# LCJebe/PCReg

Hardware: AMD Instinct MI355X
Metric: KNN Gpairs/s end-to-end (search + filters + RANSAC per step; registrations/s = 1000/ms_per_step) (higher is better)
Workload: dtype f32 (search: f16-split matrix-core candidates, exact f32 re-rank) / f64 (RANSAC)

## Files before the change

pcreg_amd/csrc/ransac.hip:

```cpp
#include "common.hpp"
#include <cfloat>
#include <cstddef>
#include <cstdio>
#include <cstdlib>

namespace pcreg {
namespace {

constexpr int kBlock = 256;
constexpr int kWavesPerBlock = 4;
constexpr int HB = 4;

struct RansacArgs {
    const double* p1; const double* p2; int ld;
    const int32_t* offsets;
    const int32_t* n_dev;
    int n_cap; int iters; int m;
    double thDist; double ratio; int refine; unsigned long long seed;
    const int32_t* sample_idx;
    int hpw;
    int hyp0g;
    double* TF;
    int32_t* cnt1; int32_t* cnt2; unsigned char* has;
    int n_hi;
// ... 817 lines not shown
                    unsigned long long bal = __ballot(in);
                    const int r3 = k3 + __popcll(bal & ((1ull << lane) - 1ull));
                    if (in && r3 < 3) {
#pragma unroll
                        for (int c = 0; c < 6; ++c) s_mom[wave][k][r3 * 6 + c] = q[c];
                    }
                    k3 += __popcll(bal);
                }
            PCREG_TILE_SWEEP_END
            if (want && ch != 3) {
                wave_sum27(acc);
#pragma unroll
                for (int e = 0; e < 27; ++e) if (lane == 0) s_mom[wave][k][e] = acc[e];
            }
        }
        __builtin_amdgcn_wave_barrier();
        {
            const bool in_round = mine && lane >= h0 && lane < h0 + HB;
            if (in_round && pass1) {
                double mom[27];
#pragma unroll
                for (int e = 0; e < 27; ++e) mom[e] = s_mom[wave][lane - h0][e];
                if (c1 == 3) {
                    double A1[3][3], A2[3][3];
#pragma unroll
                    for (int j = 0; j < 3; ++j)
#pragma unroll
                        for (int c = 0; c < 3; ++c) { A1[j][c] = mom[j * 6 + c]; A2[j][c] = mom[j * 6 + 3 + c]; }
                    v2 = fit_3pt(A1, A2, T2);
                } else {
                    v2 = fit_moments(c1, mom, o, T2);
                }
            }
        }
        {
            bool any = false;
#pragma unroll
            for (int k = 0; k < HB; ++k) any |= (__builtin_amdgcn_readlane((int)v2, min(h0 + k, 63)) != 0) && (h0 + k < nh);
            if (__syncthreads_or(any)) {
                double T[HB][12]; int cnt[HB];
#pragma unroll
                for (int k = 0; k < HB; ++k) { bcast_T(T2, min(h0 + k, 63), T[k]); pin_translation_vgpr(T[k]); cnt[k] = 0; }
                PCREG_TILE_SWEEP_BEGIN
#pragma unroll
                    for (int k = 0; k < HB; ++k) if (h0 + k < a.hpw) cnt[k] += __popcll(__ballot((sqdist(q, T[k]) < th) & act));
                PCREG_TILE_SWEEP_END
#pragma unroll
                for (int k = 0; k < HB; ++k) if (lane == h0 + k) c2 = cnt[k];
            }
        }
    }
    if (mine) {
        if (!a.refine) {
            a.cnt1[hyp0 + p] = c1; a.cnt2[hyp0 + p] = 0; a.has[hyp0 + p] = pass1;
            if (pass1) {
#pragma unroll
                for (int k = 0; k < 12; ++k) a.TF[(hyp0 + p) * 12 + k] = T1[k];
            }
        } else {
            const bool keep = v2 && c2 >= thInlr;
            a.cnt1[hyp0 + p] = c1; a.cnt2[hyp0 + p] = v2 ? c2 : 0; a.has[hyp0 + p] = keep;
            if (keep) {
#pragma unroll
                for (int k = 0; k < 12; ++k) a.TF[(hyp0 + p) * 12 + k] = T2[k];
            }
        }
    }
}


constexpr int kSW = 4, kSS = 8;
constexpr int kSPts = kSW * kSS * 64;
constexpr int kSMaxPB = 64;
#ifndef PCREG_MOM_SLOTS
#define PCREG_MOM_SLOTS 44
#endif
constexpr int kStagedMinN = 2049;
constexpr int kMomSlots = PCREG_MOM_SLOTS;
constexpr int kRec = 16;
#ifndef PCREG_SCHUNK
#define PCREG_SCHUNK 32
#endif
constexpr int kSChunk = PCREG_SCHUNK;
constexpr int kBBlk = kSS * 64, kBSeeds = 64, kBBuckets = 16, kBChunk = 4;
struct BCtr {
    int32_t lb;
    int32_t hstar;
    int32_t hist[kBBuckets], cursor[kBBuckets];
    int32_t seed_cnt[kBSeeds];
    unsigned long long stats[3];
    int32_t seed_h[kBSeeds];
};
constexpr int kBCtrClearWords = (int)(offsetof(BCtr, seed_h) / 4);

struct StagedArgs {
    RansacArgs a;
    double* T1; unsigned char* v1; unsigned char* pass1; unsigned char* v2;
    unsigned char* cert;
    double* certq;
    double* bounds;
    void* sel_ctr;
    double* bpart;
    int n_rec_blocks;
    double* mom;
    int32_t* part;
    int pb;
    unsigned long long* masks;
    int nslots_cap;
    double* rec;
    double* mpart;
    uint4* dig;
    int32_t* pass_list;
    int32_t* n_pass;
    unsigned char* dense;
    int use_lane;
    float* c32;
    int n32;
    float* T32a; float* T32b;
    int use_f32;
    float* p32;
    int32_t* perm;
    unsigned char* bkt;
    void* bctr;
};

__device__ __forceinline__ int staged_n(const RansacArgs& a) { return min(a.n_dev ? *a.n_dev : a.n_cap, a.n_cap); }

__device__ __forceinline__ void rs_records_body(const StagedArgs& sa, int block) {
    const RansacArgs& a = sa.a;
    const int n = staged_n(a);
    const int i = block * 256 + threadIdx.x;
    double m1 = 0.0, m2 = 0.0, c1m = 0.0, c2m = 0.0;
    if (i >= n && sa.use_lane && i < sa.nslots_cap * 64) {
        double* r = sa.rec + (size_t)i * kRec;
#pragma unroll
        for (int e = 0; e < kRec; ++e) r[e] = 0.0;
    }
    if (i < n) {
        Pts<false> P{a.p1, a.p2, a.ld, nullptr, n};
        double o[6], q[6];
        P.load(0, o); P.load(i, q);
        m1 = q[0] * q[0] + q[1] * q[1] + q[2] * q[2];
        m2 = q[3] * q[3] + q[4] * q[4] + q[5] * q[5];
        if (sa.use_f32 || sa.use_lane) {
            double v[6];
#pragma unroll
            for (int c = 0; c < 6; ++c) { v[c] = q[c] - o[c]; if (sa.use_f32) sa.c32[(size_t)c * sa.n32 + i] = (float)v[c]; }
            c1m = v[0] * v[0] + v[1] * v[1] + v[2] * v[2];
            c2m = v[3] * v[3] + v[4] * v[4] + v[5] * v[5];
        }
        if (sa.use_lane) {
            const double d0 = q[0] - o[0], d1 = q[1] - o[1], d2 = q[2] - o[2];
            const double m0 = q[3] - o[3], m1_ = q[4] - o[4], m2_ = q[5] - o[5];
            double* r = sa.rec + (size_t)i * kRec;
            r[0] = d0; r[1] = d1; r[2] = d2; r[3] = m0; r[4] = m1_; r[5] = m2_;
            r[6] = m0 * d0; r[7] = m0 * d1; r[8] = m0 * d2;
            r[9] = m1_ * d0; r[10] = m1_ * d1; r[11] = m1_ * d2;
            r[12] = m2_ * d0; r[13] = m2_ * d1; r[14] = m2_ * d2; r[15] = 0.0;
        }
    }
#pragma unroll
    for (int o_ = 32; o_ > 0; o_ >>= 1) {
        m1 = fmax(m1, __shfl_xor(m1, o_)); m2 = fmax(m2, __shfl_xor(m2, o_));
        c1m = fmax(c1m, __shfl_xor(c1m, o_)); c2m = fmax(c2m, __shfl_xor(c2m, o_));
    }
    __shared__ double s_mx[4][4];
    if ((threadIdx.x & 63) == 0) { const int w = threadIdx.x >> 6; s_mx[w][0] = m1; s_mx[w][1] = m2; s_mx[w][2] = c1m; s_mx[w][3] = c2m; }
// ... 285 lines not shown
    __syncthreads();
    for (int pb = blockIdx.x; pb * kSPts < n; pb += gridDim.x) {
        float q[kSS][6];
        const int ibase = pb * kSPts + wave * kSS * 64 + lane;
#pragma unroll
        for (int s = 0; s < kSS; ++s) {
            const int i = ibase + s * 64;
            const bool act = i < n;
            const int ii = act ? i : 0;
#pragma unroll
            for (int c = 0; c < 6; ++c) q[s][c] = sa.c32[(size_t)c * sa.n32 + ii];
            if (!act) q[s][0] = __builtin_nanf("");
        }
        rs_i32x16 RA, RB;
#define PCREG_ROW_LOAD(R, H) { const float* rp_ = T32 + (size_t)min((H), h1 - 1) * 16; asm volatile("s_load_dwordx16 %0, %1, 0x0" : "=&s"(R) : "s"(rp_)); }
#define PCREG_ROW_WAIT(R) asm volatile("s_waitcnt lgkmcnt(0)" : "+s"(R))
#define PCREG_SCORE_HYP(H, R)                                                                                      \
        if ((vmask[((H) - h0) >> 6] >> (((H) - h0) & 63)) & 1ull) {                                \
            float T[12];                                                                                           \
            _Pragma("unroll") for (int k = 0; k < 12; ++k) { const int w_ = R[k]; T[k] = __int_as_float(w_); }                 \
            const int wlo_ = R[12], whi_ = R[13]; const float thlo = __int_as_float(wlo_), thhi = __int_as_float(whi_);          \
            unsigned long long b[kSS], band = 0ull;                                                                \
            _Pragma("unroll") for (int s = 0; s < kSS; ++s) {                                                      \
                const float d = sqdist32(q[s], T);                                                                 \
                b[s] = __ballot(d < thlo);                                                                         \
                band |= __ballot(d <= thhi) ^ b[s];       \
            }                                                                                                      \
            if (band != 0ull) {       \
                double T64[12];       \
                _Pragma("unroll") for (int k = 0; k < 12; ++k) T64[k] = TT[(size_t)(H) * 12 + k];    \
                _Pragma("unroll 1") for (int s = 0; s < kSS; ++s) {       \
                    const int i = ibase + s * 64;                         \
                    const bool act = i < n;                                                                        \
                    const int ii = act ? i : 0;                                                                    \
                    float qq[6];                                                                                   \
                    _Pragma("unroll") for (int c = 0; c < 6; ++c) qq[c] = sa.c32[(size_t)c * sa.n32 + ii];         \
                    if (!act) qq[0] = __builtin_nanf("");                                                          \
                    const float d = sqdist32(qq, T);                                                               \
                    if ((__ballot(d <= thhi) ^ __ballot(d < thlo)) != 0ull) {                     \
                        double p[6];                                                                               \
                        _Pragma("unroll") for (int c = 0; c < 3; ++c) { p[c] = a.p1[ii + (size_t)c * a.ld]; p[3 + c] = a.p2[ii + (size_t)c * a.ld]; } \
                        const unsigned long long bb = __ballot((sqdist(p, T64) < th) & act);                       \
                        _Pragma("unroll") for (int s2 = 0; s2 < kSS; ++s2) if (s2 == s) b[s2] = bb;                \
                    }                                                                                              \
                }                                                                                                  \
            }                                                                                                      \
            int cnt = 0;                                                                                           \
            int mine_lo = 0, mine_hi = 0;                                                                          \
            _Pragma("unroll") for (int s = 0; s < kSS; ++s) {                                                      \
                cnt += __popcll(b[s]);                                                                             \
                if (EMIT) {                                                               \
                    asm volatile("v_writelane_b32 %0, %1, %2" : "+v"(mine_lo) : "s"((int)(unsigned)b[s]), "n"(s)); \
                    asm volatile("v_writelane_b32 %0, %1, %2" : "+v"(mine_hi) : "s"((int)(unsigned)(b[s] >> 32)), "n"(s)); \
                }                                                                                                  \
            }                                                                                                      \
            if (lane == 0) s_cnt[wave][(H) - h0] += cnt;                                                           \
            if (EMIT && lane < kSS)                            \
                sa.masks[(size_t)(H) * sa.nslots_cap + (size_t)pb * (kSPts / 64) + wave * kSS + lane] =            \
                    ((unsigned long long)(unsigned)mine_hi << 32) | (unsigned)mine_lo;                             \
        }
        PCREG_ROW_LOAD(RA, h0)
        PCREG_ROW_WAIT(RA);
        for (int h = h0; h < h1; h += 2) {
            PCREG_ROW_LOAD(RB, h + 1)
            PCREG_SCORE_HYP(h, RA)
            PCREG_ROW_WAIT(RB); PCREG_ROW_LOAD(RA, h + 2)
            if (h + 1 < h1) { PCREG_SCORE_HYP(h + 1, RB) }
            PCREG_ROW_WAIT(RA);
        }
#undef PCREG_SCORE_HYP
#undef PCREG_ROW_WAIT
#undef PCREG_ROW_LOAD
    }
    __syncthreads();
    for (int hl = threadIdx.x; hl < h1 - h0; hl += kSW * 64) {
        int c = 0;
#pragma unroll
        for (int w = 0; w < kSW; ++w) c += s_cnt[w][hl];
        if (acc) { if (c) atomicAdd(&acc[h0 + hl], c); } else sa.part[(size_t)blockIdx.x * a.iters + h0 + hl] = c;
    }
}


__device__ __forceinline__ void rs_load_block(const StagedArgs& sa, const float* __restrict__ x32, int base, int n, float (&q)[kSS][6]) {
    const int lane = threadIdx.x & 63;
#pragma unroll
    for (int s = 0; s < kSS; ++s) {
        const int i = base + s * 64 + lane;
        const bool act = i < n;
        const int ii = act ? i : 0;
#pragma unroll
        for (int c = 0; c < 6; ++c) q[s][c] = x32[(size_t)c * sa.n32 + ii];
        if (!act) q[s][0] = __builtin_nanf("");
    }
}
__device__ __forceinline__ int rs_block_count(const StagedArgs& sa, const float* __restrict__ x32, const int32_t* __restrict__ perm,
                                              int base, int n, const float (&q)[kSS][6], const float (&T)[12], float thlo, float thhi,
                                              int h) {
    const RansacArgs& a = sa.a;
    const int lane = threadIdx.x & 63;
    unsigned long long b[kSS], band = 0ull;
#pragma unroll
    for (int s = 0; s < kSS; ++s) {
        const float d = sqdist32(q[s], T);
        b[s] = __ballot(d < thlo);
        band |= __ballot(d <= thhi) ^ b[s];
    }
    if (band != 0ull) {
        double T64[12];
#pragma unroll
        for (int k = 0; k < 12; ++k) T64[k] = a.TF[(size_t)h * 12 + k];
#pragma unroll 1
        for (int s = 0; s < kSS; ++s) {
            const int i = base + s * 64 + lane;
            const bool act = i < n;
            const int ii = act ? i : 0;
            float qq[6];
#pragma unroll
            for (int c = 0; c < 6; ++c) qq[c] = x32[(size_t)c * sa.n32 + ii];
            if (!act) qq[0] = __builtin_nanf("");
            const float d = sqdist32(qq, T);
            if ((__ballot(d <= thhi) ^ __ballot(d < thlo)) != 0ull) {
                const int oi = perm ? perm[ii] : ii;
                double p[6];
#pragma unroll
                for (int c = 0; c < 3; ++c) { p[c] = a.p1[oi + (size_t)c * a.ld]; p[3 + c] = a.p2[oi + (size_t)c * a.ld]; }
                const unsigned long long bb = __ballot((sqdist(p, T64) < a.thDist) & act);
#pragma unroll
                for (int s2 = 0; s2 < kSS; ++s2) if (s2 == s) b[s2] = bb;
            }
        }
    }
    int cnt = 0;
#pragma unroll
    for (int s = 0; s < kSS; ++s) cnt += __popcll(b[s]);
    return cnt;
}

__device__ __forceinline__ unsigned long long rs_cnt1_key(const StagedArgs& sa, int lo, int hi) {
    unsigned long long key = 0ull;
#pragma unroll 4
    for (int p = lo + (int)(threadIdx.x & 63); p < hi; p += 64) {
        const unsigned char v = sa.v2[p];
        const unsigned long long k = ((unsigned long long)(unsigned)sa.a.cnt1[p] << 32) | (unsigned)(0xFFFFFFFFu - (unsigned)p);
        key = v && k > key ? k : key;
    }
#pragma unroll
    for (int o = 32; o > 0; o >>= 1) { const unsigned long long ot = __shfl_xor(key, o); key = ot > key ? ot : key; }
    return key;
}
__device__ __forceinline__ int rs_key_index(unsigned long long key) { return key ? (int)(0xFFFFFFFFu - (unsigned)(key & 0xFFFFFFFFull)) : -1; }

__device__ __forceinline__ int rs_order_bucket(float d, float th) {
    if (!(d < th) || !(th < 3.0e38f)) return 0;
    const int k = (int)((th - d) * ((float)(kBBuckets - 1) / th));
    return 1 + min(kBBuckets - 2, max(k, 0));
}

__global__ __launch_bounds__(256) void rs_bprep_kernel(StagedArgs sa, int n_seed_wg, int S, int nbc) {
    const RansacArgs& a = sa.a;
    BCtr* bc = (BCtr*)sa.bctr;
    const int n = staged_n(a);
    const int lane = threadIdx.x & 63, wave = threadIdx.x >> 6;
    if ((int)blockIdx.x < n_seed_wg) {
        const int u = blockIdx.x * 4 + wave;
        const int s = u / nbc, blk = u - s * nbc;
        if (s >= S || (blk > 0 && blk * kBBlk >= n)) return;
        const int lo = (int)((long long)s * a.iters / S), hi = (int)((long long)(s + 1) * a.iters / S);
        const int h = rs_key_index(rs_cnt1_key(sa, lo, hi));
        if (blk == 0 && lane == 0) bc->seed_h[s] = h;
        if (h < 0 || blk * kBBlk >= n) return;
        float q[kSS][6];
        rs_load_block(sa, sa.c32, blk * kBBlk, n, q);
        const float* row = sa.T32b + (size_t)h * 16;
        float T[12];
#pragma unroll
        for (int k = 0; k < 12; ++k) T[k] = row[k];
        const int c = rs_block_count(sa, sa.c32, nullptr, blk * kBBlk, n, q, T, row[12], row[13], h);
        if (lane == 0 && c) atomicAdd(&bc->seed_cnt[s], c);
        return;
    }
    const int ob = blockIdx.x - n_seed_wg;
    __shared__ unsigned long long s_key[4];
    __shared__ int s_hist[kBBuckets];
    if (threadIdx.x < kBBuckets) s_hist[threadIdx.x] = 0;
    {
        unsigned long long k = 0ull;
        const int n4 = a.iters >> 2;
        const int4* c4 = (const int4*)a.cnt1;
        const unsigned* v4 = (const unsigned*)sa.v2;
#pragma unroll 4
        for (int p4 = threadIdx.x; p4 < n4; p4 += 256) {
            const int4 c = c4[p4];
            const unsigned v = v4[p4];
            const int cc[4] = {c.x, c.y, c.z, c.w};
#pragma unroll
            for (int e = 0; e < 4; ++e) {
                const unsigned p = (unsigned)(4 * p4 + e);
                const unsigned long long ke = ((v >> (8 * e)) & 0xFFu) ? ((unsigned long long)(unsigned)cc[e] << 32) | (0xFFFFFFFFu - p) : 0ull;
                k = ke > k ? ke : k;
            }
        }
        for (int p = 4 * n4 + (int)threadIdx.x; p < a.iters; p += 256)
            if (sa.v2[p]) { const unsigned long long ke = ((unsigned long long)(unsigned)a.cnt1[p] << 32) | (0xFFFFFFFFu - (unsigned)p); k = ke > k ? ke : k; }
#pragma unroll
        for (int o = 32; o > 0; o >>= 1) { const unsigned long long ot = __shfl_xor(k, o); k = ot > k ? ot : k; }
        if (lane == 0) s_key[wave] = k;
    }
    __syncthreads();
    unsigned long long key = s_key[0];
#pragma unroll
    for (int w = 1; w < 4; ++w) key = s_key[w] > key ? s_key[w] : key;
    const int hs = rs_key_index(key);
    if (ob == 0) {
        if (threadIdx.x == 0) bc->hstar = hs;
        if ((int)threadIdx.x >= S && threadIdx.x < kBSeeds) bc->seed_h[threadIdx.x] = -1;
    }
    const int i = ob * 256 + threadIdx.x;
    if (i < n) {
        int bk = 0;
        if (hs >= 0) {
            float q[6], T[12];
#pragma unroll
            for (int c = 0; c < 6; ++c) q[c] = sa.c32[(size_t)c * sa.n32 + i];
#pragma unroll
            for (int k = 0; k < 12; ++k) T[k] = sa.T32b[(size_t)hs * 16 + k];
            bk = rs_order_bucket(sqdist32(q, T), (float)a.thDist);
        }
        sa.bkt[i] = (unsigned char)bk;
        atomicAdd(&s_hist[bk], 1);
    }
    __syncthreads();
    if (threadIdx.x < kBBuckets && s_hist[threadIdx.x]) atomicAdd(&bc->hist[threadIdx.x], s_hist[threadIdx.x]);
}

__global__ __launch_bounds__(256) void rs_bscatter_kernel(StagedArgs sa) {
    BCtr* bc = (BCtr*)sa.bctr;
    const int n = staged_n(sa.a);
    __shared__ int s_cnt[kBBuckets], s_off[kBBuckets];
    if (threadIdx.x < kBBuckets) s_cnt[threadIdx.x] = 0;
    __syncthreads();
    const int i = blockIdx.x * 256 + threadIdx.x;
    int bk = 0, r = 0;
    if (i < n) { bk = sa.bkt[i]; r = atomicAdd(&s_cnt[bk], 1); }
    __syncthreads();
    if (threadIdx.x < kBBuckets) {
        int off = 0;
        for (int k = 0; k < (int)threadIdx.x; ++k) off += bc->hist[k];
        s_off[threadIdx.x] = off + (s_cnt[threadIdx.x] ? atomicAdd(&bc->cursor[threadIdx.x], s_cnt[threadIdx.x]) : 0);
    }
    __syncthreads();
    if (i < n) {
        const int pos = s_off[bk] + r;
#pragma unroll
        for (int c = 0; c < 6; ++c) sa.p32[(size_t)c * sa.n32 + pos] = sa.c32[(size_t)c * sa.n32 + i];
        sa.perm[pos] = i;
    }
}

template <int C>
__global__ __launch_bounds__(64) void rs_bounded_kernel(StagedArgs sa, unsigned long long* __restrict__ stats) {
    static_assert(C >= 1 && C <= 64, "one lane per refit");
    const RansacArgs& a = sa.a;
    BCtr* bc = (BCtr*)sa.bctr;
    const int n = staged_n(a);
    const int lane = threadIdx.x;
    const int thInlr = matlab_round_i(a.ratio * (double)n);
    const int h0 = blockIdx.x * C, hl = h0 + lane;
    const bool mine = lane < C && hl < a.iters;
    const int nb = (n + kBBlk - 1) / kBBlk;
    const int sh = bc->seed_h[lane], sc = bc->seed_cnt[lane];
    int lb = sh >= 0 ? sc : 0;
#pragma unroll
    for (int o = 32; o > 0; o >>= 1) lb = max(lb, __shfl_xor(lb, o));
    bool live = mine && sa.v2[hl] != 0;
    const unsigned long long exist = __ballot(live);
    int seedc = -1;
    for (int s = 0; s < kBSeeds; ++s) {
        const int hs = __builtin_amdgcn_readlane(sh, s), cs = __builtin_amdgcn_readlane(sc, s);
        if (hs == hl) seedc = cs;
    }
    if (live && seedc >= 0) { a.cnt2[hl] = seedc; live = false; }
    unsigned long long active = __ballot(live);
    const unsigned long long seeded = exist & ~active;
    float comp[14];
#pragma unroll
    for (int k = 0; k < 14; ++k) comp[k] = live ? sa.T32b[(size_t)hl * 16 + k] : 0.0f;
    int in_v = 0;
    unsigned long long units = 0ull;
    float qa[kSS][6], qb[kSS][6];
    if (active != 0ull && nb > 0) rs_load_block(sa, sa.p32, 0, n, qa);
    int lbr0 = lb, lbr1 = lb;
    auto step = [&](int blk, const float (&cur)[kSS][6], float (&nxt)[kSS][6], int& lbr) {
        if (blk + 1 < nb) rs_load_block(sa, sa.p32, (blk + 1) * kBBlk, n, nxt);
        const int base = blk * kBBlk;
        for (unsigned long long m = active; m != 0ull; m &= m - 1ull) {
            const int j = __builtin_ctzll(m);
            float T[12];
#pragma unroll
            for (int k = 0; k < 12; ++k) T[k] = __int_as_float(__builtin_amdgcn_readlane(__float_as_int(comp[k]), j));
            const float thlo = __int_as_float(__builtin_amdgcn_readlane(__float_as_int(comp[12]), j));
            const float thhi = __int_as_float(__builtin_amdgcn_readlane(__float_as_int(comp[13]), j));
            const int c = rs_block_count(sa, sa.p32, sa.perm, base, n, cur, T, thlo, thhi, h0 + j);
            in_v += lane == j ? c : 0;
        }
        units += (unsigned long long)__popcll(active);
        lb = max(lb, lbr);
        lbr = __hip_atomic_load(&bc->lb, __ATOMIC_RELAXED, __HIP_MEMORY_SCOPE_AGENT);
        const int out_v = min(n, base + kBBlk) - in_v;
        const bool stop = ((active >> lane) & 1ull) && out_v > n - lb && (in_v >= thInlr || out_v > n - thInlr);
        if (stop) a.cnt2[hl] = in_v >= thInlr ? thInlr : 0;
        active &= ~__ballot(stop);
    };
    for (int blk = 0; blk < nb && active != 0ull; blk += 2) {
        step(blk, qa, qb, lbr0);
        if (blk + 1 < nb && active != 0ull) step(blk + 1, qb, qa, lbr1);
    }
    const bool full = (active >> lane) & 1ull;
    if (full) a.cnt2[hl] = in_v;
    int mx = full ? in_v : 0;
#pragma unroll
    for (int o = 32; o > 0; o >>= 1) mx = max(mx, __shfl_xor(mx, o));
    if (lane == 0 && active != 0ull && mx > lb) __hip_atomic_fetch_max(&bc->lb, mx, __ATOMIC_RELAXED, __HIP_MEMORY_SCOPE_AGENT);
    if (stats && lane == 0) {
        if (blockIdx.x == 0) atomicAdd(&stats[0], 1ull);
        atomicAdd(&stats[1], units + (unsigned long long)__popcll(seeded) * (unsigned long long)nb);
        atomicAdd(&stats[2], (unsigned long long)__popcll(exist) * (unsigned long long)nb);
    }
}

constexpr int kHB32 = 4;
typedef unsigned rs_u32x2 __attribute__((ext_vector_type(2)));

template <int CTRL>
__device__ __forceinline__ double dpp_f64(double v) {
    const int lo = __builtin_amdgcn_mov_dpp(__double2loint(v), CTRL, 0xF, 0xF, false);
    const int hi = __builtin_amdgcn_mov_dpp(__double2hiint(v), CTRL, 0xF, 0xF, false);
    return __hiloint2double(hi, lo);
}
__device__ __forceinline__ double swap32_add(double A, double B) {
    const rs_u32x2 r0 = __builtin_amdgcn_permlane32_swap((unsigned)__double2loint(A), (unsigned)__double2loint(B), false, false);
    const rs_u32x2 r1 = __builtin_amdgcn_permlane32_swap((unsigned)__double2hiint(A), (unsigned)__double2hiint(B), false, false);
    return __hiloint2double((int)r1[0], (int)r0[0]) + __hiloint2double((int)r1[1], (int)r0[1]);
}
__device__ __forceinline__ double swap16_add(double A, double B) {
    const rs_u32x2 r0 = __builtin_amdgcn_permlane16_swap((unsigned)__double2loint(A), (unsigned)__double2loint(B), false, false);
    const rs_u32x2 r1 = __builtin_amdgcn_permlane16_swap((unsigned)__double2hiint(A), (unsigned)__double2hiint(B), false, false);
    return __hiloint2double((int)r1[0], (int)r0[0]) + __hiloint2double((int)r1[1], (int)r0[1]);
}
__device__ __forceinline__ double wave_sum15_scatter(const double (&v)[15]) {
    const int lane = threadIdx.x & 63;
    double r1[8], r2[4], r3[2];
#pragma unroll
    for (int j = 0; j < 8; ++j) r1[j] = swap32_add(v[j], j < 7 ? v[j < 7 ? 8 + j : 14] : 0.0);
#pragma unroll
    for (int j = 0; j < 4; ++j) r2[j] = swap16_add(r1[j], r1[4 + j]);
    const bool b3 = lane & 8, b2 = lane & 4;
#pragma unroll
    for (int j = 0; j < 2; ++j) r3[j] = (b3 ? r2[2 + j] : r2[j]) + dpp_f64<0x128>(b3 ? r2[j] : r2[2 + j]);
    double r = (b2 ? r3[1] : r3[0]) + dpp_f64<0x1B>(dpp_f64<0x141>(b2 ? r3[0] : r3[1]));
    r += dpp_f64<0x4E>(r);
    r += dpp_f64<0xB1>(r);
    return r;
}
__device__ __forceinline__ void mom15_add(double (&m)[15], const double (&q)[6]) {
    m[0] += q[0]; m[1] += q[1]; m[2] += q[2]; m[3] += q[3]; m[4] += q[4]; m[5] += q[5];
    m[6]  = fma(q[3], q[0], m[6]);  m[7]  = fma(q[3], q[1], m[7]);  m[8]  = fma(q[3], q[2], m[8]);
    m[9]  = fma(q[4], q[0], m[9]);  m[10] = fma(q[4], q[1], m[10]); m[11] = fma(q[4], q[2], m[11]);
    m[12] = fma(q[5], q[0], m[12]); m[13] = fma(q[5], q[1], m[13]); m[14] = fma(q[5], q[2], m[14]);
}
__device__ bool fit_moments15(int N, const double (&mom)[15], const double (&o)[6], double (&T)[12]) {
    if (N < 4) return false;
    const double inv = 1.0 / (double)N;
    const double cdp[3] = {mom[0] * inv, mom[1] * inv, mom[2] * inv};
    const double cmp_[3] = {mom[3] * inv, mom[4] * inv, mom[5] * inv};
    double H[3][3];
#pragma unroll
    for (int i = 0; i < 3; ++i)
#pragma unroll
        for (int j = 0; j < 3; ++j) H[i][j] = mom[6 + i * 3 + j] - (double)N * cmp_[i] * cdp[j];
    const double cd[3] = {cdp[0] + o[0], cdp[1] + o[1], cdp[2] + o[2]};
    const double cm[3] = {cmp_[0] + o[3], cmp_[1] + o[4], cmp_[2] + o[5]};
    return polar_to_T(H, cd, cm, T);
}
__device__ __forceinline__ double ld_coherent(const double* p) { return __hip_atomic_load(p, __ATOMIC_RELAXED, __HIP_MEMORY_SCOPE_AGENT); }

struct Hyp32Lds { const double* c64; const float* c32; int np; int ns; };
typedef float rs_f32x2 __attribute__((ext_vector_type(2)));

__device__ __forceinline__ float sqdist32r(const float (&q)[6], const float (&T)[12]) {
    float ux = q[0] - T[9], uy = q[1] - T[10], uz = q[2] - T[11];
    ux = __builtin_fmaf(q[5], -T[2], ux); uy = __builtin_fmaf(q[5], -T[5], uy); uz = __builtin_fmaf(q[5], -T[8], uz);
    ux = __builtin_fmaf(q[4], -T[1], ux); uy = __builtin_fmaf(q[4], -T[4], uy); uz = __builtin_fmaf(q[4], -T[7], uz);
    ux = __builtin_fmaf(q[3], -T[0], ux); uy = __builtin_fmaf(q[3], -T[3], uy); uz = __builtin_fmaf(q[3], -T[6], uz);
    return __builtin_fmaf(uz, uz, __builtin_fmaf(uy, uy, ux * ux));
}
__device__ __forceinline__ rs_f32x2 sqdist32r_x2(const rs_f32x2 (&q)[6], const rs_f32x2 (&P)[6]) {
    rs_f32x2 ux, uy, uz, d;
    asm("v_pk_add_f32 %0, %4, %10 op_sel_hi:[1,0] neg_lo:[0,1] neg_hi:[0,1]\n\t"
        "v_pk_add_f32 %1, %5, %10 op_sel:[0,1] op_sel_hi:[1,1] neg_lo:[0,1] neg_hi:[0,1]\n\t"
        "v_pk_add_f32 %2, %6, %11 op_sel_hi:[1,0] neg_lo:[0,1] neg_hi:[0,1]\n\t"
        "v_pk_fma_f32 %0, %9, %11, %0 op_sel:[0,1,0] op_sel_hi:[1,1,1] neg_lo:[0,1,0] neg_hi:[0,1,0]\n\t"
        "v_pk_fma_f32 %1, %9, %12, %1 op_sel_hi:[1,0,1] neg_lo:[0,1,0] neg_hi:[0,1,0]\n\t"
        "v_pk_fma_f32 %2, %9, %12, %2 op_sel:[0,1,0] op_sel_hi:[1,1,1] neg_lo:[0,1,0] neg_hi:[0,1,0]\n\t"
        "v_pk_fma_f32 %0, %8, %13, %0 op_sel_hi:[1,0,1] neg_lo:[0,1,0] neg_hi:[0,1,0]\n\t"
        "v_pk_fma_f32 %1, %8, %13, %1 op_sel:[0,1,0] op_sel_hi:[1,1,1] neg_lo:[0,1,0] neg_hi:[0,1,0]\n\t"
        "v_pk_fma_f32 %2, %8, %14, %2 op_sel_hi:[1,0,1] neg_lo:[0,1,0] neg_hi:[0,1,0]\n\t"
        "v_pk_fma_f32 %0, %7, %14, %0 op_sel:[0,1,0] op_sel_hi:[1,1,1] neg_lo:[0,1,0] neg_hi:[0,1,0]\n\t"
        "v_pk_fma_f32 %1, %7, %15, %1 op_sel_hi:[1,0,1] neg_lo:[0,1,0] neg_hi:[0,1,0]\n\t"
        "v_pk_fma_f32 %2, %7, %15, %2 op_sel:[0,1,0] op_sel_hi:[1,1,1] neg_lo:[0,1,0] neg_hi:[0,1,0]\n\t"
        "v_pk_mul_f32 %3, %0, %0\n\t"
// ... 1204 lines not shown
    if (ws_bytes < need) { set_error("ransac workspace too small: %zu < %zu", ws_bytes, need); return PCREG_E_WORKSPACE; }
    size_t h = (size_t)o.iterNum * (size_t)B;
    RansacArgs a{};
    a.p1 = p1; a.p2 = p2; a.ld = ld; a.offsets = offsets; a.n_dev = n_dev; a.n_cap = n_cap;
    a.iters = o.iterNum; a.m = o.minPtNum; a.thDist = o.thDist; a.ratio = o.thInlrRatio;
    a.refine = o.REFINE != 0; a.seed = o.seed; a.sample_idx = sample_idx_dev; a.hyp0g = hyp_begin;
    a.n_hi = 0x7FFFFFFF; a.n_lo = -1;
    a.TF = lay.TF; a.cnt1 = lay.cnt1; a.cnt2 = lay.cnt2; a.has = lay.has;
    long long total = (long long)o.iterNum * B;
    void* sel_ctr = nullptr;
    SelFinish sel_fin{nullptr, nullptr, 0};
    bool fold_finish = false;
    if (debug_flag(kDbgRansacResidentF64) && n_cap > 0 && (size_t)n_cap * 48 <= (offsets ? (size_t)152 * 1024 : (size_t)64 * 1024)) {
        size_t lds = (size_t)n_cap * 48;
        int hpw = 64;
        while (hpw > 8 && total / hpw < 256LL * 4 * 2) hpw >>= 1;
        a.hpw = hpw;
        if (offsets && lds > 64 * 1024) { lds = 32 * 1024; a.n_hi = (int)(lds / 48); }
        const int pb4 = hpw * kWavesPerBlock;
        hipLaunchKernelGGL(ransac_hyp_kernel, dim3((o.iterNum + pb4 - 1) / pb4, B), dim3(kBlock), lds, st, a);
    } else if (n_cap > 0 && n_cap <= (offsets ? kHyp32BatchCap : kHyp32Classes[kHyp32NClasses - 1])) {
        int hpw = 64;
        while (hpw > 8 && total / hpw < 256LL * 4 * 2) hpw >>= 1;
        a.hpw = hpw;
        a.msc = lay.msc;
        const int c = n_cap <= kHyp32Classes[0] ? 0 : 1;
        a.n_lo = -1; a.n_hi = std::min(n_cap, kHyp32Classes[c]);
        const int nw = kHyp32Waves[c], per_block = hpw * nw;
        const dim3 grid((o.iterNum + per_block - 1) / per_block, B);
        const int rc = nw == 8 ? launch_hyp32<8>(a, grid, hyp32_lds_bytes(a.n_hi, nw), st) : launch_hyp32<16>(a, grid, hyp32_lds_bytes(a.n_hi, nw), st);
        if (rc != PCREG_OK) return rc;
        const int lo = a.n_hi;
        if (n_cap > lo) {
            a.n_lo = lo; a.n_hi = -1;
            const int pb4 = hpw * kWavesPerBlock;
            hipLaunchKernelGGL(ransac_hyp_kernel, dim3((o.iterNum + pb4 - 1) / pb4, B), dim3(kBlock), 0, st, a);
        }
    } else if (B == 1 && !offsets && staged_pays(n_cap, o.iterNum) && !debug_flag(kDbgRansacFused)) {
        StagedArgs sa = lay.sa;
        sel_ctr = sa.sel_ctr;
        sa.use_lane = a.refine && !debug_flag(kDbgRansacNoLane);
        sa.use_f32 = !debug_flag(kDbgRansacF64Score);
        int pb = (n_cap + kSPts - 1) / kSPts; if (pb > kSMaxPB) pb = kSMaxPB; if (pb < 1) pb = 1;
        sa.pb = pb;
        int hpw = (int)((total + 250LL * kTW - 1) / (250LL * kTW));
        if (hpw < 1) hpw = 1;
        if (hpw > 16) hpw = 16;
        a.hpw = hpw;
        sa.a = a;
        const int it = o.iterNum;
        const dim3 sgrid(pb, (it + kSChunk - 1) / kSChunk);
        const int n_fit = (it + 255) / 256;
        hipLaunchKernelGGL(rs_stage1_kernel, dim3((unsigned)(n_fit + sa.n_rec_blocks)), dim3(256), 0, st, sa, n_fit);
        const int n_t32 = (it + 255) / 256, n_dig = sa.use_lane ? (int)staged_slots_cap(n_cap) * 2 : 0;
        hipLaunchKernelGGL(rs_stage2_kernel, dim3((unsigned)(n_t32 + n_dig)), dim3(256), 0, st, sa, (const double*)sa.T1, sa.T32a, n_t32, sa.dig);
        if (sa.use_f32) {
            if (sa.use_lane)
                hipLaunchKernelGGL(rs_score32_kernel<true>, sgrid, dim3(kSW * 64), 0, st, sa, (const double*)sa.T1, (const float*)sa.T32a, (const unsigned char*)sa.v1, (int32_t*)nullptr);
            else
                hipLaunchKernelGGL(rs_score32_kernel<false>, sgrid, dim3(kSW * 64), 0, st, sa, (const double*)sa.T1, (const float*)sa.T32a, (const unsigned char*)sa.v1, (int32_t*)nullptr);
        } else if (sa.use_lane) {
            hipLaunchKernelGGL(rs_score_kernel<true>, sgrid, dim3(kSW * 64), 0, st, sa, (const double*)sa.T1, (const unsigned char*)sa.v1);
        } else {
            hipLaunchKernelGGL(rs_score_kernel<false>, sgrid, dim3(kSW * 64), 0, st, sa, (const double*)sa.T1, (const unsigned char*)sa.v1);
        }
        hipLaunchKernelGGL(rs_pass1_kernel, dim3((it + 255) / 256), dim3(256), 0, st, sa);
        if (a.refine) {
            if (sa.use_lane)
                hipLaunchKernelGGL(rs_moments_mfma_kernel, dim3((it + kMmWaves * kMmRows - 1) / (kMmWaves * kMmRows), (unsigned)staged_chunks_cap(n_cap)), dim3(kMmWaves * 64), 0, st, sa,
                                   (const uint4*)sa.dig, (const unsigned long long*)sa.masks);
            hipLaunchKernelGGL(rs_moments_kernel, dim3((it + hpw * kTW - 1) / (hpw * kTW)), dim3(kTBlock), 0, st, sa);
            hipLaunchKernelGGL(rs_fit2_kernel, dim3((it + 63) / 64), dim3(64), 0, st, sa);
            fold_finish = !part && n_cap <= kSelBlocks * kSelPerThread * kSelThreads;
            const int p2mode = debug_flag(kDbgRansacPass2);
            const bool bounded = fold_finish && sa.use_f32 && !iter_inl_ref && p2mode != 1 && (p2mode == 2 || bounded_pays(n_cap, it));
            if (bounded) {
                const int S = std::min(kBSeeds, it), nbc = (n_cap + kBBlk - 1) / kBBlk;
                const int n_seed_wg = (S * nbc + 3) / 4, n_ord_wg = (n_cap + 255) / 256;
                unsigned long long* stats = ransac_stats_dev();
                hipLaunchKernelGGL(rs_bprep_kernel, dim3((unsigned)(n_seed_wg + n_ord_wg)), dim3(256), 0, st, sa, n_seed_wg, S, nbc);
                hipLaunchKernelGGL(rs_bscatter_kernel, dim3((unsigned)n_ord_wg), dim3(256), 0, st, sa);
#ifdef PCREG_EXPERIMENTS
                const int dbg = PCREG_EXP_ENV("PCREG_RANSAC_DEBUG", 0), chunk = PCREG_EXP_ENV("PCREG_RANSAC_BCHUNK", kBChunk);
                unsigned long long* kst = dbg ? ((BCtr*)sa.bctr)->stats : stats;
                if (chunk == 8) hipLaunchKernelGGL(rs_bounded_kernel<8>, dim3((unsigned)((it + 7) / 8)), dim3(64), 0, st, sa, kst);
                else if (chunk == 2) hipLaunchKernelGGL(rs_bounded_kernel<2>, dim3((unsigned)((it + 1) / 2)), dim3(64), 0, st, sa, kst);
                else hipLaunchKernelGGL(rs_bounded_kernel<kBChunk>, dim3((unsigned)((it + kBChunk - 1) / kBChunk)), dim3(64), 0, st, sa, kst);
                if (dbg) {
                    unsigned long long u[3] = {0, 0, 0};
                    PCREG_HIP(hipMemcpyAsync(u, kst, sizeof u, hipMemcpyDeviceToHost, st));
                    PCREG_HIP(hipStreamSynchronize(st));
                    fprintf(stderr, "[pcreg] ransac bounded pass 2: iters=%d n_cap=%d chunk=%d (refit, block) units scanned %llu of %llu (%.4f)\n", it, n_cap,
                            chunk == 8 || chunk == 2 ? chunk : kBChunk, u[1], u[2], u[2] ? (double)u[1] / (double)u[2] : 0.0);
                }
#else
                hipLaunchKernelGGL(rs_bounded_kernel<kBChunk>, dim3((unsigned)((it + kBChunk - 1) / kBChunk)), dim3(64), 0, st, sa, stats);
#endif
            } else if (sa.use_f32)
                hipLaunchKernelGGL(rs_score32_kernel<false>, sgrid, dim3(kSW * 64), 0, st, sa, (const double*)a.TF, (const float*)sa.T32b, (const unsigned char*)sa.v2,
                                   fold_finish ? a.cnt2 : (int32_t*)nullptr);
            else
                hipLaunchKernelGGL(rs_score_kernel<false>, sgrid, dim3(kSW * 64), 0, st, sa, (const double*)a.TF, (const unsigned char*)sa.v2);
            if (fold_finish) { sel_fin.part = sa.use_f32 ? nullptr : sa.part; sel_fin.v2 = sa.v2; sel_fin.pb = sa.pb; }
            else hipLaunchKernelGGL(rs_finish_kernel, dim3((it + 255) / 256), dim3(256), 0, st, sa);
        }
    } else {
        int hpw = (int)((total + 250LL * kTW - 1) / (250LL * kTW));
        if (hpw < 1) hpw = 1;
        if (hpw > 16) hpw = 16;
        a.hpw = hpw;
        int per_block = hpw * kTW;
        dim3 grid((o.iterNum + per_block - 1) / per_block, B);
        hipLaunchKernelGGL(ransac_hyp_tiled_kernel, grid, dim3(kTBlock), 0, st, a);
    }
    PCREG_HIP(hipGetLastError());
    if (sel_ctr && !part && n_cap <= kSelBlocks * kSelPerThread * kSelThreads) {
        int per_block = 4 * kSelThreads;
        if ((n_cap + per_block - 1) / per_block > kSelBlocks) per_block = ((n_cap + kSelBlocks - 1) / kSelBlocks + kSelThreads - 1) / kSelThreads * kSelThreads;
        const int nb = std::max(1, (n_cap + per_block - 1) / per_block);
        hipLaunchKernelGGL(ransac_select_multi_kernel, dim3(nb), dim3(kSelThreads), 0, st, a, out, inlier_idx, (SelCtr*)sel_ctr, per_block, sel_fin);
    }
    else if (n_cap >= 8192) hipLaunchKernelGGL(ransac_select_kernel<1024>, dim3(B), dim3(1024), 0, st, a, out, inlier_idx, part);
    else hipLaunchKernelGGL(ransac_select_kernel<kBlock>, dim3(B), dim3(kBlock), 0, st, a, out, inlier_idx, part);
    PCREG_HIP(hipGetLastError());
    if (iter_inl) PCREG_HIP(hipMemcpyAsync(iter_inl, a.cnt1, h * sizeof(int32_t), hipMemcpyDeviceToDevice, st));
    if (iter_inl_ref) PCREG_HIP(hipMemcpyAsync(iter_inl_ref, a.cnt2, h * sizeof(int32_t), hipMemcpyDeviceToDevice, st));
    return PCREG_OK;
}

int launch_ransac(const double* p1, const double* p2, int ld, const int32_t* offsets, const int32_t* n_dev,
                  int n_cap, int B, const pcreg_ransac_opts& o, const int32_t* sample_idx_dev,
                  pcreg_dev_ransac_result* out, int32_t* inlier_idx, int32_t* iter_inl, int32_t* iter_inl_ref,
                  void* ws, size_t ws_bytes, hipStream_t st) {
    return launch_ransac_impl(p1, p2, ld, offsets, n_dev, n_cap, B, o, sample_idx_dev, out, inlier_idx, iter_inl, iter_inl_ref,
                              ws, ws_bytes, st, 0, nullptr);
}

int launch_ransac_partial(const double* p1, const double* p2, int ld, const int32_t* n_dev, int n_cap,
                          const pcreg_ransac_opts& o, const int32_t* sample_idx_dev, int hyp_begin, int hyp_count,
                          pcreg_dev_ransac_part* part, void* ws, size_t ws_bytes, hipStream_t st) {
    PCREG_ARG(hyp_begin >= 0 && hyp_count >= 0 && hyp_begin + hyp_count <= o.iterNum);
    if (hyp_count == 0) { PCREG_HIP(hipMemsetAsync(part, 0, sizeof(pcreg_dev_ransac_part), st)); return PCREG_OK; }
    pcreg_ransac_opts ol = o;
    ol.iterNum = hyp_count;
    return launch_ransac_impl(p1, p2, ld, nullptr, n_dev, n_cap, 1, ol, sample_idx_dev, nullptr, nullptr, nullptr, nullptr,
                              ws, ws_bytes, st, hyp_begin, part);
}

int launch_ransac_finish(const double* p1, const double* p2, int ld, const int32_t* n_dev, int n_cap,
                         const pcreg_ransac_opts& o, const pcreg_dev_ransac_part* combined,
                         pcreg_dev_ransac_result* out, int32_t* inlier_idx, hipStream_t st, int n_parts) {
    PCREG_ARG(n_parts >= 1);
    RansacArgs a{};
    a.p1 = p1; a.p2 = p2; a.ld = ld; a.n_dev = n_dev; a.n_cap = n_cap; a.thDist = o.thDist; a.ratio = o.thInlrRatio;
    if (n_cap >= 8192) hipLaunchKernelGGL(ransac_finish_kernel<1024>, dim3(1), dim3(1024), 0, st, a, combined, n_parts, out, inlier_idx);
    else hipLaunchKernelGGL(ransac_finish_kernel<kBlock>, dim3(1), dim3(kBlock), 0, st, a, combined, n_parts, out, inlier_idx);
    PCREG_HIP(hipGetLastError());
    return PCREG_OK;
}

int launch_estimate_transform(const double* p1, const double* p2, int n, int ld, double* T16_dev,
                              int32_t* empty_dev, hipStream_t st) {
    hipLaunchKernelGGL(estimate_transform_kernel, dim3(1), dim3(64), 0, st, p1, p2, n, ld, T16_dev, empty_dev);
    PCREG_HIP(hipGetLastError());
    return PCREG_OK;
}

int launch_refine_by_distance(const double* p1, const double* p2, const int32_t* n_dev, int cap, int ld, double maxDist,
                              double* T16_dev, int32_t* info_dev, hipStream_t st) {
    hipLaunchKernelGGL(refine_by_distance_kernel, dim3(1), dim3(64), 0, st, p1, p2, n_dev, cap, ld, maxDist, T16_dev, info_dev);
    PCREG_HIP(hipGetLastError());
    return PCREG_OK;
}

int launch_estimate_transform_indexed(const double* p1, const double* p2, int ld, const int32_t* idx, int32_t idx_base, const int32_t* n_idx_dev,
                                      int cap, double* T16_dev, int32_t* info_dev, hipStream_t st) {
    hipLaunchKernelGGL(estimate_transform_indexed_kernel, dim3(1), dim3(64), 0, st, p1, p2, ld, idx, (int)idx_base, n_idx_dev, cap, T16_dev, info_dev);
    PCREG_HIP(hipGetLastError());
    return PCREG_OK;
// ... 23 lines not shown
```

Measured before the change: 123,700.

## Split bounded RANSAC scoring blocks across four waves per workgroup

The bounded pass-2 kernel now runs four waves per workgroup. Each wave scores a different 512-point block for the same small set of refit hypotheses, and per-round counts and the lower bound are combined through shared memory with a barrier. Point loads are also vectorised to float4 per lane, which reorders rows within a block. This targets latency in what was a single-wave serial scan, at the cost of a barrier each round and coarser early-stop granularity, since all four blocks are scanned before a stop check.

```diff
diff --git a/pcreg_amd/csrc/ransac.hip b/pcreg_amd/csrc/ransac.hip
--- a/pcreg_amd/csrc/ransac.hip
+++ b/pcreg_amd/csrc/ransac.hip
@@ -923,7 +923,8 @@
 #define PCREG_SCHUNK 32
 #endif
 constexpr int kSChunk = PCREG_SCHUNK;
-constexpr int kBBlk = kSS * 64, kBSeeds = 64, kBBuckets = 16, kBChunk = 4;
+constexpr int kBBlk = kSS * 64, kBSeeds = 64, kBBuckets = 16, kBChunk = 4, kBWaves = 4;
+constexpr bool kBPrefetch = true;
 struct BCtr {
     int32_t lb;
     int32_t hstar;
@@ -1375,16 +1376,20 @@
 }
 
 
+__device__ __forceinline__ int rs_block_row(int s, int lane) { return 256 * (s >> 2) + 4 * lane + (s & 3); }
 __device__ __forceinline__ void rs_load_block(const StagedArgs& sa, const float* __restrict__ x32, int base, int n, float (&q)[kSS][6]) {
+    static_assert(kSS == 8 && kSPts % kBBlk == 0, "two float4 per lane and coordinate");
     const int lane = threadIdx.x & 63;
 #pragma unroll
-    for (int s = 0; s < kSS; ++s) {
-        const int i = base + s * 64 + lane;
-        const bool act = i < n;
-        const int ii = act ? i : 0;
-#pragma unroll
-        for (int c = 0; c < 6; ++c) q[s][c] = x32[(size_t)c * sa.n32 + ii];
-        if (!act) q[s][0] = __builtin_nanf("");
+    for (int g = 0; g < 2; ++g) {
+        const int i0 = base + 256 * g + 4 * lane;
+#pragma unroll
+        for (int c = 0; c < 6; ++c) {
+            const float4 v = ((const float4*)(x32 + (size_t)c * sa.n32 + base + 256 * g))[lane];
+            q[4 * g][c] = v.x; q[4 * g + 1][c] = v.y; q[4 * g + 2][c] = v.z; q[4 * g + 3][c] = v.w;
+        }
+#pragma unroll
+        for (int e = 0; e < 4; ++e) if (i0 + e >= n) q[4 * g + e][0] = __builtin_nanf("");
     }
 }
 __device__ __forceinline__ int rs_block_count(const StagedArgs& sa, const float* __restrict__ x32, const int32_t* __restrict__ perm,
@@ -1405,7 +1410,7 @@
         for (int k = 0; k < 12; ++k) T64[k] = a.TF[(size_t)h * 12 + k];
 #pragma unroll 1
         for (int s = 0; s < kSS; ++s) {
-            const int i = base + s * 64 + lane;
+            const int i = base + rs_block_row(s, lane);
             const bool act = i < n;
             const int ii = act ? i : 0;
             float qq[6];
@@ -1551,17 +1556,21 @@
     }
 }
 
-template <int C>
-__global__ __launch_bounds__(64) void rs_bounded_kernel(StagedArgs sa, unsigned long long* __restrict__ stats) {
+template <int C, int W, bool PF>
+__global__ __launch_bounds__(64 * W) void rs_bounded_kernel(StagedArgs sa, unsigned long long* __restrict__ stats) {
     static_assert(C >= 1 && C <= 64, "one lane per refit");
+    static_assert(W >= 1 && W <= 16, "waves of one workgroup");
     const RansacArgs& a = sa.a;
     BCtr* bc = (BCtr*)sa.bctr;
     const int n = staged_n(a);
-    const int lane = threadIdx.x;
+    const int lane = threadIdx.x & 63, wave = threadIdx.x >> 6;
     const int thInlr = matlab_round_i(a.ratio * (double)n);
     const int h0 = blockIdx.x * C, hl = h0 + lane;
     const bool mine = lane < C && hl < a.iters;
     const int nb = (n + kBBlk - 1) / kBBlk;
+    __shared__ int s_cnt[2][W][C];
+    __shared__ int s_lb[2];
+    __shared__ unsigned long long s_units[W];
     const int sh = bc->seed_h[lane], sc = bc->seed_cnt[lane];
     int lb = sh >= 0 ? sc : 0;
 #pragma unroll
@@ -1573,7 +1582,7 @@
         const int hs = __builtin_amdgcn_readlane(sh, s), cs = __builtin_amdgcn_readlane(sc, s);
         if (hs == hl) seedc = cs;
     }
-    if (live && seedc >= 0) { a.cnt2[hl] = seedc; live = false; }
+    if (live && seedc >= 0) { if (wave == 0) a.cnt2[hl] = seedc; live = false; }
     unsigned long long active = __ballot(live);
     const unsigned long long seeded = exist & ~active;
     float comp[14];
@@ -1582,44 +1591,68 @@
     int in_v = 0;
     unsigned long long units = 0ull;
     float qa[kSS][6], qb[kSS][6];
-    if (active != 0ull && nb > 0) rs_load_block(sa, sa.p32, 0, n, qa);
+    if (PF && active != 0ull && wave < nb) rs_load_block(sa, sa.p32, wave * kBBlk, n, qa);
     int lbr0 = lb, lbr1 = lb;
-    auto step = [&](int blk, const float (&cur)[kSS][6], float (&nxt)[kSS][6], int& lbr) {
-        if (blk + 1 < nb) rs_load_block(sa, sa.p32, (blk + 1) * kBBlk, n, nxt);
-        const int base = blk * kBBlk;
-        for (unsigned long long m = active; m != 0ull; m &= m - 1ull) {
-            const int j = __builtin_ctzll(m);
-            float T[12];
-#pragma unroll
-            for (int k = 0; k < 12; ++k) T[k] = __int_as_float(__builtin_amdgcn_readlane(__float_as_int(comp[k]), j));
-            const float thlo = __int_as_float(__builtin_amdgcn_readlane(__float_as_int(comp[12]), j));
-            const float thhi = __int_as_float(__builtin_amdgcn_readlane(__float_as_int(comp[13]), j));
-            const int c = rs_block_count(sa, sa.p32, sa.perm, base, n, cur, T, thlo, thhi, h0 + j);
-            in_v += lane == j ? c : 0;
-        }
-        units += (unsigned long long)__popcll(active);
-        lb = max(lb, lbr);
-        lbr = __hip_atomic_load(&bc->lb, __ATOMIC_RELAXED, __HIP_MEMORY_SCOPE_AGENT);
-        const int out_v = min(n, base + kBBlk) - in_v;
+    auto step = [&](int r, float (&cur)[kSS][6], float (&nxt)[kSS][6], int& lbr) {
+        const int blk = W * r + wave, base = blk * kBBlk;
+        if (PF) { if (blk + W < nb) rs_load_block(sa, sa.p32, (blk + W) * kBBlk, n, nxt); }
+        else if (blk < nb) rs_load_block(sa, sa.p32, base, n, cur);
+        int c_v = 0;
+        if (blk < nb) {
+            for (unsigned long long m = active; m != 0ull; m &= m - 1ull) {
+                const int j = __builtin_ctzll(m);
+                float T[12];
+#pragma unroll
+                for (int k = 0; k < 12; ++k) T[k] = __int_as_float(__builtin_amdgcn_readlane(__float_as_int(comp[k]), j));
+                const float thlo = __int_as_float(__builtin_amdgcn_readlane(__float_as_int(comp[12]), j));
+                const float thhi = __int_as_float(__builtin_amdgcn_readlane(__float_as_int(comp[13]), j));
+                const int c = rs_block_count(sa, sa.p32, sa.perm, base, n, cur, T, thlo, thhi, h0 + j);
+                c_v += lane == j ? c : 0;
+            }
+            units += (unsigned long long)__popcll(active);
+        }
+        if (lane < C) s_cnt[r & 1][wave][lane] = c_v;
+        if (wave == 0) {
+            if (lane == 0) s_lb[r & 1] = lbr;
+            lbr = __hip_atomic_load(&bc->lb, __ATOMIC_RELAXED, __HIP_MEMORY_SCOPE_AGENT);
+        }
+        __syncthreads();
+        if (lane < C) {
+#pragma unroll
+            for (int w = 0; w < W; ++w) in_v += s_cnt[r & 1][w][lane];
+        }
+        lb = max(lb, s_lb[r & 1]);
+        const int out_v = min(n, (W * r + W) * kBBlk) - in_v;
         const bool stop = ((active >> lane) & 1ull) && out_v > n - lb && (in_v >= thInlr || out_v > n - thInlr);
-        if (stop) a.cnt2[hl] = in_v >= thInlr ? thInlr : 0;
+        if (stop && wave == 0) a.cnt2[hl] = in_v >= thInlr ? thInlr : 0;
         active &= ~__ballot(stop);
     };
-    for (int blk = 0; blk < nb && active != 0ull; blk += 2) {
-        step(blk, qa, qb, lbr0);
-        if (blk + 1 < nb && active != 0ull) step(blk + 1, qb, qa, lbr1);
+    const int nr = (nb + W - 1) / W;
+    for (int r = 0; r < nr && active != 0ull; r += 2) {
+        step(r, qa, PF ? qb : qa, lbr0);
+        if (r + 1 < nr && active != 0ull) step(r + 1, PF ? qb : qa, qa, lbr1);
     }
     const bool full = (active >> lane) & 1ull;
+    if (lane == 0) s_units[wave] = units;
+    __syncthreads();
+    if (wave != 0) return;
     if (full) a.cnt2[hl] = in_v;
     int mx = full ? in_v : 0;
 #pragma unroll
     for (int o = 32; o > 0; o >>= 1) mx = max(mx, __shfl_xor(mx, o));
     if (lane == 0 && active != 0ull && mx > lb) __hip_atomic_fetch_max(&bc->lb, mx, __ATOMIC_RELAXED, __HIP_MEMORY_SCOPE_AGENT);
     if (stats && lane == 0) {
+        units = 0ull;
+#pragma unroll
+        for (int w = 0; w < W; ++w) units += s_units[w];
         if (blockIdx.x == 0) atomicAdd(&stats[0], 1ull);
         atomicAdd(&stats[1], units + (unsigned long long)__popcll(seeded) * (unsigned long long)nb);
         atomicAdd(&stats[2], (unsigned long long)__popcll(exist) * (unsigned long long)nb);
     }
+}
+template <int C, int W, bool PF>
+static void rs_bounded_launch(const StagedArgs& sa, int it, unsigned long long* stats, hipStream_t st) {
+    hipLaunchKernelGGL((rs_bounded_kernel<C, W, PF>), dim3((unsigned)((it + C - 1) / C)), dim3(64 * W), 0, st, sa, stats);
 }
 
 constexpr int kHB32 = 4;
@@ -2990,19 +3023,24 @@
                 hipLaunchKernelGGL(rs_bscatter_kernel, dim3((unsigned)n_ord_wg), dim3(256), 0, st, sa);
 #ifdef PCREG_EXPERIMENTS
                 const int dbg = PCREG_EXP_ENV("PCREG_RANSAC_DEBUG", 0), chunk = PCREG_EXP_ENV("PCREG_RANSAC_BCHUNK", kBChunk);
+                const int waves = PCREG_EXP_ENV("PCREG_RANSAC_BWAVES", kBWaves), pf = PCREG_EXP_ENV("PCREG_RANSAC_BPREFETCH", kBPrefetch ? 1 : 0);
                 unsigned long long* kst = dbg ? ((BCtr*)sa.bctr)->stats : stats;
-                if (chunk == 8) hipLaunchKernelGGL(rs_bounded_kernel<8>, dim3((unsigned)((it + 7) / 8)), dim3(64), 0, st, sa, kst);
-                else if (chunk == 2) hipLaunchKernelGGL(rs_bounded_kernel<2>, dim3((unsigned)((it + 1) / 2)), dim3(64), 0, st, sa, kst);
-                else hipLaunchKernelGGL(rs_bounded_kernel<kBChunk>, dim3((unsigned)((it + kBChunk - 1) / kBChunk)), dim3(64), 0, st, sa, kst);
+#define PCREG_BOUNDED_CASE(C_, W_)                                                                                                 \
+                if (chunk == C_ && waves == W_) { if (pf) rs_bounded_launch<C_, W_, true>(sa, it, kst, st); else rs_bounded_launch<C_, W_, false>(sa, it, kst, st); } else
+                PCREG_BOUNDED_CASE(2, 1) PCREG_BOUNDED_CASE(2, 2) PCREG_BOUNDED_CASE(2, 4)
+                PCREG_BOUNDED_CASE(4, 1) PCREG_BOUNDED_CASE(4, 2) PCREG_BOUNDED_CASE(4, 4)
+                if (chunk == 8) rs_bounded_launch<8, 1, true>(sa, it, kst, st);
+                else { fprintf(stderr, "[pcreg] PCREG_RANSAC_BCHUNK=%d PCREG_RANSAC_BWAVES=%d: not built, the default runs\n", chunk, waves); rs_bounded_launch<kBChunk, kBWaves, kBPrefetch>(sa, it, kst, st); }
+#undef PCREG_BOUNDED_CASE
                 if (dbg) {
                     unsigned long long u[3] = {0, 0, 0};
                     PCREG_HIP(hipMemcpyAsync(u, kst, sizeof u, hipMemcpyDeviceToHost, st));
                     PCREG_HIP(hipStreamSynchronize(st));
-                    fprintf(stderr, "[pcreg] ransac bounded pass 2: iters=%d n_cap=%d chunk=%d (refit, block) units scanned %llu of %llu (%.4f)\n", it, n_cap,
-                            chunk == 8 || chunk == 2 ? chunk : kBChunk, u[1], u[2], u[2] ? (double)u[1] / (double)u[2] : 0.0);
+                    fprintf(stderr, "[pcreg] ransac bounded pass 2: iters=%d n_cap=%d chunk=%d waves=%d prefetch=%d (refit, block) units scanned %llu of %llu (%.4f)\n",
+                            it, n_cap, chunk, waves, pf, u[1], u[2], u[2] ? (double)u[1] / (double)u[2] : 0.0);
                 }
 #else
-                hipLaunchKernelGGL(rs_bounded_kernel<kBChunk>, dim3((unsigned)((it + kBChunk - 1) / kBChunk)), dim3(64), 0, st, sa, stats);
+                rs_bounded_launch<kBChunk, kBWaves, kBPrefetch>(sa, it, stats, st);
 #endif
             } else if (sa.use_f32)
                 hipLaunchKernelGGL(rs_score32_kernel<false>, sgrid, dim3(kSW * 64), 0, st, sa, (const double*)a.TF, (const float*)sa.T32b, (const unsigned char*)sa.v2,
```

After: 120,000. 0.97x the previous value.
